# TinfoilHat0/Defending-Against-Backdoors-with-Robust-Learning-Rate

Measured on NVIDIA H100. Metric: fl_rounds_per_sec, higher is better.
Workload: dtype bf16

## Files before the change

### defending-against-backdoors-with-robust-learning-rate_b200/ops/csrc/gemm.cu

```cuda
#include <cuda.h>
#include <stdlib.h>

#include "common.cuh"
#include "gemm.h"
#include "stem_gather.cuh"
#include "wgmma.cuh"

namespace rlr {

using namespace wg;

constexpr int BM = 128;
constexpr int BK = 64;
constexpr int kConsumers = 256;
constexpr int kThreads = kConsumers + 64;
constexpr int kEpiThreads = kConsumers;

template <int BN, int kOcc = 2>
struct TileCfg {
    static_assert(kOcc != 1 || BN == 128, "the one-wave configuration exists for the 128-wide tile");
    static constexpr int kStages = kOcc == 1 ? 6 : kOcc == 3 ? (BN == 64 ? 3 : 2) : (BN == 64 ? 4 : 3);
    static constexpr int kABytes = BM * BK * 2;
    static constexpr int kBBytes = BN * BK * 2;
    static constexpr int kStageBytes = kABytes + kBBytes;
// ... 222 lines not shown
        named_bar(1, kEpiThreads);
        if (dbg && et == 0) dbg[6] = (long long)gtimer();
        constexpr int kChunks = BN * 2 / 16;
        __nv_bfloat16* out = reinterpret_cast<__nv_bfloat16*>(p.out);
        constexpr int kIters = BM * kChunks / kEpiThreads;
        constexpr int kBatch = kIters < 8 ? kIters : 8;
#pragma unroll
        for (int it0 = 0; it0 < kIters; it0 += kBatch) {
            uint4 oldv[kBatch];
            if (p.accumulate) {
#pragma unroll
                for (int j = 0; j < kBatch; ++j) {
                    const int idx = et + (it0 + j) * kEpiThreads, r = idx / kChunks, ch = idx - r * kChunks;
                    const int gi = tail->row_index[r];
                    oldv[j] = make_uint4(0, 0, 0, 0);
                    if (gi >= 0 && col0 + ch * 8 < p.N) oldv[j] = *reinterpret_cast<const uint4*>(out + (size_t)gi * p.ldc + col0 + ch * 8);
                }
            }
#pragma unroll
            for (int j = 0; j < kBatch; ++j) {
                const int idx = et + (it0 + j) * kEpiThreads, r = idx / kChunks, ch = idx - r * kChunks;
                const int gi = tail->row_index[r];
                if (gi < 0 || col0 + ch * 8 >= p.N) continue;
                uint4 val = *reinterpret_cast<const uint4*>(staging + r * Cfg::kPitch + ch * 16);
                if (p.accumulate) {
                    const __nv_bfloat162* o2 = reinterpret_cast<const __nv_bfloat162*>(&oldv[j]);
                    __nv_bfloat162* v2 = reinterpret_cast<__nv_bfloat162*>(&val);
#pragma unroll
                    for (int q = 0; q < 4; ++q) {
                        const float2 a = __bfloat1622float2(v2[q]), b = __bfloat1622float2(o2[q]);
                        v2[q] = __floats2bfloat162_rn(a.x + b.x, a.y + b.y);
                    }
                }
                *reinterpret_cast<uint4*>(out + (size_t)gi * p.ldc + col0 + ch * 8) = val;
            }
        }
        if (kStats) {
            named_bar(1, kEpiThreads);
            for (int i = et; i < 2 * BN; i += kEpiThreads)
                if (col0 + (i % BN) < p.N)
                    atomicAdd(p.stats + (size_t)(blockIdx.x % kStatSlots) * 2 * p.N + (i < BN ? 0 : p.N) + col0 + (i % BN), red[i]);
        }
        }
    }
}

typedef CUresult (*EncodeTiledFn)(CUtensorMap*, CUtensorMapDataType, cuuint32_t, void*, const cuuint64_t*, const cuuint64_t*,
                                  const cuuint32_t*, const cuuint32_t*, CUtensorMapInterleave, CUtensorMapSwizzle,
                                  CUtensorMapL2promotion, CUtensorMapFloatOOBfill);

static EncodeTiledFn get_encode_fn() {
    static EncodeTiledFn fn = nullptr;
    if (!fn) {
        void* f = nullptr;
        cudaDriverEntryPointQueryResult q;
        if (cudaGetDriverEntryPoint("cuTensorMapEncodeTiled", &f, cudaEnableDefault, &q) != cudaSuccess || !f) return nullptr;
        fn = reinterpret_cast<EncodeTiledFn>(f);
    }
    return fn;
}

cudaError_t make_tmap_bf16(CUtensorMap* map, const void* base, int rank, const uint64_t* dims, const uint64_t* strides_bytes,
                           const uint32_t* box, const uint32_t* elem_strides = nullptr) {
    EncodeTiledFn fn = get_encode_fn();
    if (!fn) return cudaErrorNotSupported;
    cuuint64_t gd[5], gs[4];
    cuuint32_t bx[5], es[5];
    for (int i = 0; i < rank; ++i) {
        gd[i] = dims[i];
        es[i] = elem_strides ? elem_strides[i] : 1;
        bx[i] = box[i] * es[i];
        if (bx[i] > 256 || es[i] < 1 || es[i] > 8) return cudaErrorInvalidValue;
    }
    for (int i = 0; i + 1 < rank; ++i) gs[i] = strides_bytes[i];
    const CUresult r = fn(map, CU_TENSOR_MAP_DATA_TYPE_BFLOAT16, (cuuint32_t)rank, const_cast<void*>(base), gd, gs, bx, es,
                          CU_TENSOR_MAP_INTERLEAVE_NONE, CU_TENSOR_MAP_SWIZZLE_128B, CU_TENSOR_MAP_L2_PROMOTION_L2_256B,
                          CU_TENSOR_MAP_FLOAT_OOB_FILL_NONE);
    return r == CUDA_SUCCESS ? cudaSuccess : cudaErrorInvalidValue;
}

template <int BN>
cudaError_t launch_persistent_bn(const CUtensorMap& tmA, const CUtensorMap& tmB, const ConvGemmParams& p, int m_tiles, int num_sms,
                                 cudaStream_t st, int occ = 1);

static int g_occ3 = -1;
void set_conv_occ3(int level) { g_occ3 = level < 0 ? 0 : (level > 1 ? 1 : level); }
static int conv_occ3() {
    if (g_occ3 < 0) { const char* e = getenv("RLR_CONV_OCC3"); set_conv_occ3(e ? atoi(e) : 1); }
    return g_occ3;
}

template <int BN, int kOcc>
static cudaError_t launch_bn_occ(const CUtensorMap& tmA, const CUtensorMap& tmB, const CUtensorMap& tmC, const ConvGemmParams& p, int m_tiles,
                                 cudaStream_t st) {
    using Cfg = TileCfg<BN, kOcc>;
    static bool configured = false;
    if (!configured) {
        RLR_CUDA_CHECK(cudaFuncSetAttribute(umma_conv_gemm_kernel<BN, false, false, kOcc>, cudaFuncAttributeMaxDynamicSharedMemorySize, Cfg::kSmemBytes));
        RLR_CUDA_CHECK(cudaFuncSetAttribute(umma_conv_gemm_kernel<BN, false, true, kOcc>, cudaFuncAttributeMaxDynamicSharedMemorySize, Cfg::kSmemBytes));
        configured = true;
    }
    dim3 grid(m_tiles, (p.N + BN - 1) / BN);
    if (p.b_mn) return launch_kernel(umma_conv_gemm_kernel<BN, false, true, kOcc>, grid, dim3(kThreads), Cfg::kSmemBytes, st, tmA, tmB, tmC, p);
    return launch_kernel(umma_conv_gemm_kernel<BN, false, false, kOcc>, grid, dim3(kThreads), Cfg::kSmemBytes, st, tmA, tmB, tmC, p);
}

static int sm_count() {
    static const int sms = [] {
        int dev = 0, n = 0;
        if (cudaGetDevice(&dev) != cudaSuccess || cudaDeviceGetAttribute(&n, cudaDevAttrMultiProcessorCount, dev) != cudaSuccess) return 132;
        return n;
    }();
    return sms;
}

static int g_persistent = -1;
void set_persistent_conv(int on) { g_persistent = on ? 1 : 0; }

static int persistent_sms() {
    if (g_persistent < 0) { const char* e = getenv("RLR_PERSISTENT_CONV"); g_persistent = (e && atoi(e) > 0) ? 1 : 0; }
    if (!g_persistent) return 0;
    static const int sms = [] {
        int dev = 0, n = 0;
        if (cudaGetDevice(&dev) != cudaSuccess || cudaDeviceGetAttribute(&n, cudaDevAttrMultiProcessorCount, dev) != cudaSuccess) return 0;
        return n;
    }();
    return sms;
}

static int g_split_prod = -1;
void set_conv_split_producer(int on) { g_split_prod = on ? 1 : 0; }
static long long* g_trace = nullptr;
void set_conv_trace(long long* buf) { g_trace = buf; }
long long* conv_trace_buf() { return g_trace; }

static int g_tma_store = -1;
void set_conv_tma_store(int on) { g_tma_store = on ? 1 : 0; }
static bool tma_store_enabled() {
    if (g_tma_store < 0) { const char* e = getenv("RLR_TMA_STORE"); g_tma_store = (e && atoi(e) == 0) ? 0 : 1; }
    return g_tma_store != 0;
}
static cudaError_t make_out_tmap(CUtensorMap* tmC, const ConvGemmParams& p) {
    if (p.ldc % 8) return cudaErrorInvalidValue;
    if (p.mode == 1) {
        const uint64_t d[4] = {(uint64_t)p.N, (uint64_t)p.Wo, (uint64_t)p.Ho, (uint64_t)p.NB};
        const uint64_t s[3] = {(uint64_t)p.out_stride * p.ldc * 2, (uint64_t)p.out_stride * p.OutW * p.ldc * 2, (uint64_t)p.OutH * p.OutW * p.ldc * 2};
        const uint32_t b[4] = {64, (uint32_t)p.TW, (uint32_t)p.TH, (uint32_t)p.TN};
        const char* base = reinterpret_cast<const char*>(p.out) + ((size_t)p.out_ph * p.OutW + p.out_pw) * p.ldc * 2;
        return make_tmap_bf16(tmC, base, 4, d, s, b);
    }
    const uint64_t d[2] = {(uint64_t)p.N, (uint64_t)p.M}, s[1] = {(uint64_t)p.ldc * 2};
    const uint32_t b[2] = {64, BM};
    return make_tmap_bf16(tmC, p.out, 2, d, s, b);
}

static void finish_params(ConvGemmParams& p, CUtensorMap& tmC) {
    p.dbg = g_trace;
    {
        static const int epi_slots = [] { const char* e = getenv("RLR_EPI_STAT_SLOTS"); int v = e ? atoi(e) : 2; return v < 1 ? 1 : (v > kStatSlots ? kStatSlots : v); }();
        p.stat_slots = epi_slots;
    }
    p.tma_store = 0;
    if (tma_store_enabled() && !p.accumulate && ((reinterpret_cast<uintptr_t>(p.out) & 15) == 0) && make_out_tmap(&tmC, p) == cudaSuccess)
        p.tma_store = 1;
    if (g_split_prod < 0) { const char* e = getenv("RLR_SPLIT_PRODUCER"); g_split_prod = (e && atoi(e) == 0) ? 0 : 1; }
    p.split_prod = (g_split_prod && !p.b_src) ? 1 : 0;
}

template <int BN>
static cudaError_t launch_bn(const CUtensorMap& tmA, const CUtensorMap& tmB, const CUtensorMap& tmC, const ConvGemmParams& p, int m_tiles,
                             cudaStream_t st) {
    using Cfg = TileCfg<BN>;
    if (p.b_src && !p.stats && p.N <= BN) {
        static const int stem_persistent = [] { const char* e = getenv("RLR_STEM_PERSISTENT"); return e ? atoi(e) : 2; }();
        if (stem_persistent && m_tiles >= 2 * sm_count())
            return launch_persistent_bn<BN>(tmA, tmB, p, m_tiles, sm_count(), st, stem_persistent == 2 ? 2 : 1);
    }
    if (!p.stats && !p.b_src && persistent_sms() > 0 && m_tiles * ((p.N + BN - 1) / BN) > persistent_sms())
        return launch_persistent_bn<BN>(tmA, tmB, p, m_tiles, persistent_sms(), st);
    if constexpr (BN == 64)
        if ((!p.stats || p.tma_store) && conv_occ3() >= 1) return launch_bn_occ<BN, 3>(tmA, tmB, tmC, p, m_tiles, st);
    static bool configured = false;
    if (!configured) {
        RLR_CUDA_CHECK(cudaFuncSetAttribute(umma_conv_gemm_kernel<BN, false, false>, cudaFuncAttributeMaxDynamicSharedMemorySize, Cfg::kSmemBytes));
        RLR_CUDA_CHECK(cudaFuncSetAttribute(umma_conv_gemm_kernel<BN, true, false>, cudaFuncAttributeMaxDynamicSharedMemorySize, Cfg::kSmemBytes));
        RLR_CUDA_CHECK(cudaFuncSetAttribute(umma_conv_gemm_kernel<BN, false, true>, cudaFuncAttributeMaxDynamicSharedMemorySize, Cfg::kSmemBytes));
        configured = true;
    }
    dim3 grid(m_tiles, (p.N + BN - 1) / BN);
    if (p.b_mn) return launch_kernel(umma_conv_gemm_kernel<BN, false, true>, grid, dim3(kThreads), Cfg::kSmemBytes, st, tmA, tmB, tmC, p);
    if (p.stats && !p.tma_store) return launch_kernel(umma_conv_gemm_kernel<BN, true, false>, grid, dim3(kThreads), Cfg::kSmemBytes, st, tmA, tmB, tmC, p);
    return launch_kernel(umma_conv_gemm_kernel<BN, false, false>, grid, dim3(kThreads), Cfg::kSmemBytes, st, tmA, tmB, tmC, p);
}

static int pick_bn(int N) { return (N % 128 == 0) ? 128 : 64; }

static int g_one_wave = 1;
void set_conv_one_wave(int on) { g_one_wave = on ? 1 : 0; }

constexpr int kOneWaveMinKb = 24;
struct ConvTile { int bn; bool one_wave; };
static ConvTile pick_conv_tile(long long px, int m_tiles, int Cout, int num_kb, bool one_wave_ok) {
    const int sms = sm_count();
    if (g_one_wave && one_wave_ok && Cout % 128 == 0 && num_kb >= kOneWaveMinKb) {
        const int ctas = m_tiles * (Cout / 128);
        if (ctas <= sms && 10 * ctas >= 9 * sms) return {128, true};
    }
    const int bn = pick_bn(Cout);
    if (bn == 128 && ((px + BM - 1) / BM) * (Cout / 128) < sms) return {64, false};
    return {bn, false};
}

cudaError_t launch_gemm_bf16(const void* A, const void* B, void* out, int M, int N, int K, int lda, int ldb, int ldc,
                             const float* bias, int relu, int accumulate, float* stats, cudaStream_t st, const DropSpec* drop) {
    if (K % BK || N % 8 || M <= 0) return cudaErrorInvalidValue;
    if (drop && drop->thr && (accumulate || stats || ldc % 8)) return cudaErrorInvalidValue;
    const int m_tiles = (M + BM - 1) / BM;
    int bn = pick_bn(N);
    {
        static const int small64 = [] { const char* e = getenv("RLR_GEMM_SMALL_BN64"); return e ? atoi(e) : 0; }();
        if (small64 && bn == 128 && m_tiles * (N / 128) < sm_count()) bn = 64;
    }
    CUtensorMap tmA, tmB;
    {
        const uint64_t d[2] = {(uint64_t)K, (uint64_t)M}, s[1] = {(uint64_t)lda * 2};
        const uint32_t b[2] = {BK, BM};
        RLR_CUDA_CHECK(make_tmap_bf16(&tmA, A, 2, d, s, b));
    }
    {
        const uint64_t d[2] = {(uint64_t)K, (uint64_t)N}, s[1] = {(uint64_t)ldb * 2};
        const uint32_t b[2] = {BK, (uint32_t)bn};
        RLR_CUDA_CHECK(make_tmap_bf16(&tmB, B, 2, d, s, b));
    }
    ConvGemmParams p{};
    p.M = M; p.N = N; p.num_kb = K / BK; p.mode = 0; p.in_stride = 1; p.out_stride = 1;
    p.out = out; p.ldc = ldc; p.bias = bias; p.stats = stats; p.relu = relu; p.accumulate = accumulate;
    if (drop && drop->thr) p.drop = *drop;
    CUtensorMap tmC = tmA;
    finish_params(p, tmC);
    return bn == 128 ? launch_bn<128>(tmA, tmB, tmC, p, m_tiles, st) : launch_bn<64>(tmA, tmB, tmC, p, m_tiles, st);
}

cudaError_t launch_stem_gemm_bf16(const void* A, const void* W, void* out, int M, int N, int kvalid, int ldw, const float* bias, int relu,
                                  float* stats, const uint32_t* wait_flags, int wait_lo, int wait_hi, const uint32_t* wait_epoch,
                                  cudaStream_t st) {
    if (N % 8 || M <= 0 || kvalid < 1 || kvalid > BK || ldw < kvalid) return cudaErrorInvalidValue;
    if (wait_flags && (!wait_epoch || wait_lo > wait_hi || wait_lo < 0)) return cudaErrorInvalidValue;
    const int m_tiles = (M + BM - 1) / BM;
    const int bn = pick_bn(N);
    CUtensorMap tmA;
    {
        const uint64_t d[2] = {(uint64_t)BK, (uint64_t)M}, s[1] = {(uint64_t)BK * 2};
        const uint32_t b[2] = {BK, BM};
        RLR_CUDA_CHECK(make_tmap_bf16(&tmA, A, 2, d, s, b));
    }
    ConvGemmParams p{};
    p.M = M; p.N = N; p.num_kb = 1; p.mode = 0; p.in_stride = 1; p.out_stride = 1;
    p.out = out; p.ldc = N; p.bias = bias; p.stats = stats; p.relu = relu; p.accumulate = 0;
    p.b_src = reinterpret_cast<const __nv_bfloat16*>(W); p.b_ld = ldw; p.b_kvalid = kvalid;
    p.wait_flags = wait_flags; p.wait_lo = wait_lo; p.wait_hi = wait_hi; p.wait_epoch = wait_epoch;
    CUtensorMap tmC = tmA;
    finish_params(p, tmC);
// ... 56 lines not shown
```

### defending-against-backdoors-with-robust-learning-rate_b200/ops/csrc/gemm.h

```cpp
#pragma once
#include <cuda_runtime.h>
#include <cuda_bf16.h>
#include <stdint.h>

#include "dropspec.h"

namespace rlr {

constexpr int kStatSlots = 16;

struct ConvGemmParams {
    int M, N, num_kb;
    int mode;
    int cblocks;
    int TW, TH, TN;
    int Ho, Wo, NB;
    int tiles_w, tiles_h;
    int ntaps;
    int in_stride;
    int out_stride, out_ph, out_pw, OutH, OutW;
    int8_t dh[9], dw[9];
    int dn[9];
    int b_mn;
    int wtap[9];
    int wcols;
    DropSpec drop;
    int tma_store;
    int split_prod;
    long long* dbg;
    const __nv_bfloat16* b_src;
    int b_ld, b_kvalid;
    const uint32_t* wait_flags;
    int wait_lo, wait_hi;
    const uint32_t* wait_epoch;
    void* out;
    int ldc;
    const float* bias;
    float* stats;
    int stat_slots;
    int relu, accumulate;
};

cudaError_t launch_gemm_bf16(const void* A, const void* B, void* out, int M, int N, int K, int lda, int ldb, int ldc,
                             const float* bias, int relu, int accumulate, float* stats, cudaStream_t st, const DropSpec* drop = nullptr);
cudaError_t launch_stem_gemm_bf16(const void* A, const void* W, void* out, int M, int N, int kvalid, int ldw, const float* bias, int relu,
                                  float* stats, const uint32_t* wait_flags, int wait_lo, int wait_hi, const uint32_t* wait_epoch,
                                  cudaStream_t st);
void set_pdl(int on);
cudaError_t launch_gemm_splitk_bf16(const void* A, const void* B, void* out, float* ws, int M, int N, int K, const float* bias, int relu,
                                    int num_sms, cudaStream_t st, const DropSpec* drop = nullptr);
void set_persistent_conv(int on);
void set_conv_occ3(int level);
void set_conv_one_wave(int on);
void set_conv_tma_store(int on);
void set_conv_split_producer(int on);
void set_conv_trace(long long* buf);
long long* conv_trace_buf();
cudaError_t launch_conv_bf16(const void* x, const void* w, void* out, int NB, int planes, int Hin, int Win, int Cin, int Ho, int Wo,
                             int Cout, int ldc, int ntaps, const int* dh, const int* dw, const int* dplane, const float* bias,
                             int relu, int accumulate, float* stats, cudaStream_t st, const int* wtap = nullptr, int w_taps_total = 0,
                             int in_stride = 1, int out_stride = 1, int out_ph = 0, int out_pw = 0);

cudaError_t launch_conv3x3_halo_bf16(const void* x, const void* w, void* out, int NB, int Hin, int Win, int H, int W, int Cout, const float* bias,
                                     int relu, int accumulate, float* stats, int bo_mode, long long* dbg, int num_sms, cudaStream_t st);

cudaError_t launch_conv3x3_halo3_bf16(const void* x, const void* w, void* out, int NB, int H, int W, int Cout, const float* bias, int relu,
                                      int accumulate, int num_sms, cudaStream_t st);

cudaError_t launch_conv_wgrad_bf16(const void* dy, const void* x, float* dW, int NB, int planes, int Hin, int Win, int Cin, int Cin_valid,
                                   int Ho, int Wo, int Cout, int ntaps, const int* dh, const int* dw, const int* dplane, int num_sms,
                                   cudaStream_t st, int in_stride = 1);
cudaError_t launch_conv_wgrad_halo_bf16(const void* dy, const void* x, float* dW, int NB, int H, int W, int Cin_valid, int Cout,
                                        int num_sms, cudaStream_t st);
void set_wgrad_rows(int on);
void wgrad_launch_counts(long long* out);
cudaError_t launch_linear_wgrad_bf16(const void* dy, const void* x, float* dW, int B, int N, int K, int num_sms, cudaStream_t st);

cudaError_t launch_ordered_sum_f32(float* out, const float* part, int nparts, long long n, cudaStream_t st);
cudaError_t launch_ordered_sum_f64(double* out, const double* part, int nparts, long long n, cudaStream_t st);
cudaError_t launch_channel_stats(const __nv_bfloat16* x, long long M, int C, float* stats , int num_sms, cudaStream_t st,
                                 int only_sum = 0, int nslots = 1);
cudaError_t launch_bn_finalize(const float* stats, int slots, float* mean_rstd, float* running_mean, float* running_var, int C,
                               float count, float eps, float momentum, int train, cudaStream_t st);
cudaError_t launch_bn_apply(const __nv_bfloat16* x, const __nv_bfloat16* res, __nv_bfloat16* y, const float* gamma, const float* beta,
                            float* mean_rstd, long long M, int C, int relu, int fin_mode, const float* stats, int slots, float count,
                            float eps, float momentum, float* running_mean, float* running_var, int num_sms, cudaStream_t st);
cudaError_t launch_bn_bwd_reduce(const __nv_bfloat16* dy, const __nv_bfloat16* y, const __nv_bfloat16* x, const float* mean_rstd,
                                 float* dsum , long long M, int C, int relu, int num_sms, cudaStream_t st,
                                 const float* gamma = nullptr, const float* beta = nullptr, int nslots = 1);
cudaError_t launch_bn_bwd_apply(const __nv_bfloat16* dy, const __nv_bfloat16* y, const __nv_bfloat16* x, const float* gamma,
                                const float* mean_rstd, const float* dsum, __nv_bfloat16* dx, __nv_bfloat16* dres, float* dgamma,
                                float* dbeta, long long M, int C, int relu, int num_sms, cudaStream_t st, const float* beta = nullptr, int nslots = 1);
cudaError_t launch_gn_fwd(const __nv_bfloat16* x, const __nv_bfloat16* res, __nv_bfloat16* y, const float* gamma, const float* beta,
                          float* mean_rstd, int B, int HW, int C, int G, float eps, int relu, int num_sms, cudaStream_t st);
cudaError_t launch_gn_bwd(const __nv_bfloat16* dy, const __nv_bfloat16* y, const __nv_bfloat16* x, const float* gamma,
                          const float* mean_rstd, __nv_bfloat16* dx, __nv_bfloat16* dres, float* dgamma, float* dbeta, int B, int HW,
                          int C, int G, int relu, int num_sms, cudaStream_t st);
cudaError_t launch_relu_bwd(__nv_bfloat16* dy, const __nv_bfloat16* y, long long n, int num_sms, cudaStream_t st, float scale = 1.0f);
cudaError_t launch_maxpool2_fwd(const __nv_bfloat16* x, __nv_bfloat16* y, uint8_t* idx, int B, int H, int W, int C, cudaStream_t st,
                                float drop_p = 0.f, uint64_t seed = 0, const long long* step = nullptr, uint64_t stream = 0);
cudaError_t launch_maxpool2_bwd(const __nv_bfloat16* dy, const uint8_t* idx, __nv_bfloat16* dx, int B, int H, int W, int C, cudaStream_t st,
                                float drop_p, uint64_t seed, const long long* step, uint64_t stream, const __nv_bfloat16* zmask);
cudaError_t launch_avgpool_fwd(const __nv_bfloat16* x, __nv_bfloat16* y, int B, int HW, int C, cudaStream_t st);
cudaError_t launch_avgpool_bwd(const __nv_bfloat16* dy, __nv_bfloat16* dx, int B, int HW, int C, cudaStream_t st);
cudaError_t launch_dropout_fwd(const __nv_bfloat16* x, __nv_bfloat16* y, uint8_t* mask, long long n, float p, uint64_t seed,
                               const long long* step, uint64_t stream, cudaStream_t st);
cudaError_t launch_dropout_bwd(const __nv_bfloat16* dy, const uint8_t* mask, __nv_bfloat16* dx, long long n, float p, cudaStream_t st);
cudaError_t launch_space_to_depth(const __nv_bfloat16* x, __nv_bfloat16* y, int NB, int H, int W, int C, int num_sms, cudaStream_t st);
cudaError_t launch_im2col_small(const __nv_bfloat16* x, __nv_bfloat16* A, int NB, int H, int W, int C, int Ho, int Wo, int k, int pad,
                                int num_sms, cudaStream_t st);
cudaError_t launch_depth_to_space(const __nv_bfloat16* x4, __nv_bfloat16* y, int NB, int H, int W, int C, int accumulate, int plane_mask,
                                  int num_sms, cudaStream_t st);
cudaError_t launch_filter_gather_transpose(const __nv_bfloat16* w, __nv_bfloat16* wt, int Cout, int T, int Cin, int nsub, const int* taps,
                                           cudaStream_t st);
cudaError_t launch_filter_transpose(const __nv_bfloat16* w, __nv_bfloat16* wt, int Cout, int ntaps, int Cin, cudaStream_t st);
cudaError_t launch_linear_small_fwd(const __nv_bfloat16* x, const __nv_bfloat16* w, const float* bias, __nv_bfloat16* y, int B, int K,
                                    int N, int relu, cudaStream_t st);
cudaError_t launch_linear_small_fwd2(const __nv_bfloat16* x, const __nv_bfloat16* w, const float* bias, __nv_bfloat16* y, int B, int K,
                                     int N, int relu, cudaStream_t st);
cudaError_t launch_linear_small_bwd2(const __nv_bfloat16* x, const __nv_bfloat16* dy, const __nv_bfloat16* w, __nv_bfloat16* dx,
                                     float* dw, float* db, int B, int K, int N, int accumulate_dx, cudaStream_t st);
cudaError_t launch_linear_small_bwd(const __nv_bfloat16* x, const __nv_bfloat16* dy, const __nv_bfloat16* w, __nv_bfloat16* dx,
                                    float* dw, float* db, int B, int K, int N, int accumulate_dx, cudaStream_t st);

}
```

### defending-against-backdoors-with-robust-learning-rate_b200/ops/csrc/gemm_binding.cpp

```cpp
#include <torch/extension.h>
#include <ATen/cuda/CUDAContext.h>
#include <c10/cuda/CUDAGuard.h>
#include <c10/cuda/CUDAStream.h>
#include <c10/cuda/CUDACachingAllocator.h>

#include <vector>

#include "gemm.h"

namespace rlr {
void* scratch_alloc(size_t bytes, cudaStream_t st) {
    return c10::cuda::CUDACachingAllocator::raw_alloc_with_stream(bytes < 256 ? 256 : bytes, st);
}
void scratch_free(void* p) { c10::cuda::CUDACachingAllocator::raw_delete(p); }
}

namespace {
inline cudaStream_t cur_stream() { return c10::cuda::getCurrentCUDAStream().stream(); }
inline int num_sms() { return at::cuda::getCurrentDeviceProperties()->multiProcessorCount; }
inline void check(cudaError_t e, const char* what) { TORCH_CHECK(e == cudaSuccess, what, ": ", cudaGetErrorString(e)); }
template <typename T>
inline T* opt(const c10::optional<at::Tensor>& t) { return t.has_value() && t->defined() ? reinterpret_cast<T*>(t->data_ptr()) : nullptr; }
inline const __nv_bfloat16* bf(const at::Tensor& t) {
    TORCH_CHECK(t.is_cuda() && t.scalar_type() == at::kBFloat16 && t.is_contiguous(), "expected contiguous CUDA bf16 tensor");
// ... 254 lines not shown
}
void maxpool2_bwd(at::Tensor dy, at::Tensor idx, at::Tensor dx, double drop_p, int64_t drop_seed, c10::optional<at::Tensor> drop_step, int64_t drop_stream,
                  c10::optional<at::Tensor> relu_out) {
    c10::cuda::CUDAGuard g(dx.device());
    const rlr::DropSpec d = drop_spec(drop_p, drop_seed, drop_step, drop_stream);
    const bool zm = relu_out.has_value() && relu_out->defined();
    TORCH_CHECK(!zm || (relu_out->scalar_type() == at::kBFloat16 && relu_out->is_contiguous() && relu_out->numel() == dy.numel()), "relu_out must match dy");
    TORCH_CHECK(dy.is_contiguous() && dx.is_contiguous() && idx.is_contiguous() && dy.size(1) == dx.size(1) / 2 && dy.size(2) == dx.size(2) / 2);
    check(rlr::launch_maxpool2_bwd(bf(dy), (const uint8_t*)idx.data_ptr(), bfm(dx), dx.size(0), dx.size(1), dx.size(2), dx.size(3), cur_stream(),
                                   (float)drop_p, d.seed, d.step, d.stream, zm ? bf(*relu_out) : nullptr), "maxpool2_bwd");
}
void avgpool_fwd(at::Tensor x, at::Tensor y) {
    c10::cuda::CUDAGuard g(x.device());
    check(rlr::launch_avgpool_fwd(bf(x), bfm(y), x.size(0), x.size(1) * x.size(2), x.size(3), cur_stream()), "avgpool_fwd");
}
void avgpool_bwd(at::Tensor dy, at::Tensor dx) {
    c10::cuda::CUDAGuard g(dx.device());
    check(rlr::launch_avgpool_bwd(bf(dy), bfm(dx), dx.size(0), dx.size(1) * dx.size(2), dx.size(3), cur_stream()), "avgpool_bwd");
}
void dropout_fwd(at::Tensor x, at::Tensor y, at::Tensor mask, double p, int64_t seed, at::Tensor step, int64_t stream) {
    c10::cuda::CUDAGuard g(x.device());
    check(rlr::launch_dropout_fwd(bf(x), bfm(y), (uint8_t*)mask.data_ptr(), x.numel(), (float)p, (uint64_t)seed,
                                  (const long long*)step.data_ptr(), (uint64_t)stream, cur_stream()), "dropout_fwd");
}
void dropout_bwd(at::Tensor dy, at::Tensor mask, at::Tensor dx, double p) {
    c10::cuda::CUDAGuard g(dx.device());
    check(rlr::launch_dropout_bwd(bf(dy), (const uint8_t*)mask.data_ptr(), bfm(dx), dx.numel(), (float)p, cur_stream()), "dropout_bwd");
}
void space_to_depth(at::Tensor x, at::Tensor y) {
    c10::cuda::CUDAGuard g(x.device());
    check(rlr::launch_space_to_depth(bf(x), bfm(y), x.size(0), x.size(1), x.size(2), x.size(3), num_sms(), cur_stream()), "space_to_depth");
}
void im2col_small(at::Tensor x, at::Tensor A, int64_t k, int64_t pad) {
    c10::cuda::CUDAGuard g(x.device());
    const int NB = x.size(0), H = x.size(1), W = x.size(2), C = x.size(3);
    const int Ho = H + 2 * pad - k + 1, Wo = W + 2 * pad - k + 1;
    TORCH_CHECK(x.dim() == 4 && x.is_contiguous() && A.is_contiguous() && A.numel() == (int64_t)NB * Ho * Wo * 64, "im2col_small: A must be [NB*Ho*Wo, 64]");
    check(rlr::launch_im2col_small(bf(x), bfm(A), NB, H, W, C, Ho, Wo, (int)k, (int)pad, num_sms(), cur_stream()), "im2col_small");
}
void depth_to_space(at::Tensor x4, at::Tensor y, bool accumulate, int64_t plane_mask) {
    c10::cuda::CUDAGuard g(y.device());
    check(rlr::launch_depth_to_space(bf(x4), bfm(y), y.size(0), y.size(1), y.size(2), y.size(3), accumulate, (int)plane_mask, num_sms(),
                                     cur_stream()), "depth_to_space");
}
void filter_gather_transpose(at::Tensor w, at::Tensor wt, int64_t Cout, int64_t T, int64_t Cin, std::vector<int64_t> taps) {
    c10::cuda::CUDAGuard g(w.device());
    int t[9];
    TORCH_CHECK(taps.size() >= 1 && taps.size() <= 9);
    for (size_t i = 0; i < taps.size(); ++i) t[i] = (int)taps[i];
    check(rlr::launch_filter_gather_transpose(bf(w), bfm(wt), Cout, T, Cin, (int)taps.size(), t, cur_stream()), "filter_gather_transpose");
}
void filter_transpose(at::Tensor w, at::Tensor wt, int64_t Cout, int64_t ntaps, int64_t Cin) {
    c10::cuda::CUDAGuard g(w.device());
    check(rlr::launch_filter_transpose(bf(w), bfm(wt), Cout, ntaps, Cin, cur_stream()), "filter_transpose");
}
void linear_small_fwd(at::Tensor x, at::Tensor w, c10::optional<at::Tensor> bias, at::Tensor y, bool relu) {
    c10::cuda::CUDAGuard g(x.device());
    check(rlr::launch_linear_small_fwd(bf(x), bf(w), opt<const float>(bias), bfm(y), x.size(0), x.size(1), w.size(0), relu, cur_stream()), "linear_small_fwd");
}
void linear_small_bwd(at::Tensor x, at::Tensor dy, at::Tensor w, c10::optional<at::Tensor> dx, at::Tensor dw, c10::optional<at::Tensor> db,
                      bool accumulate_dx) {
    c10::cuda::CUDAGuard g(x.device());
    check(rlr::launch_linear_small_bwd(bf(x), bf(dy), bf(w), const_cast<__nv_bfloat16*>(bfo(dx)), (float*)dw.data_ptr(), opt<float>(db),
                                       x.size(0), x.size(1), w.size(0), accumulate_dx, cur_stream()), "linear_small_bwd");
}
void linear_small_fwd2(at::Tensor x, at::Tensor w, c10::optional<at::Tensor> bias, at::Tensor y, bool relu) {
    c10::cuda::CUDAGuard g(x.device());
    check(rlr::launch_linear_small_fwd2(bf(x), bf(w), opt<const float>(bias), bfm(y), x.size(0), x.size(1), w.size(0), relu, cur_stream()), "linear_small_fwd2");
}
void linear_small_bwd2(at::Tensor x, at::Tensor dy, at::Tensor w, c10::optional<at::Tensor> dx, at::Tensor dw, c10::optional<at::Tensor> db,
                       bool accumulate_dx) {
    c10::cuda::CUDAGuard g(x.device());
    check(rlr::launch_linear_small_bwd2(bf(x), bf(dy), bf(w), const_cast<__nv_bfloat16*>(bfo(dx)), (float*)dw.data_ptr(), opt<float>(db),
                                        x.size(0), x.size(1), w.size(0), accumulate_dx, cur_stream()), "linear_small_bwd2");
}
}

void register_gemm_bindings(py::module_& m) {
    m.attr("STAT_SLOTS") = rlr::kStatSlots;
    m.def("set_persistent_conv", [](bool on) { rlr::set_persistent_conv(on ? 1 : 0); });
    m.def("set_pdl", [](bool on) { rlr::set_pdl(on ? 1 : 0); });
    m.def("set_conv_occ3", [](int64_t level) { rlr::set_conv_occ3((int)level); });
    m.def("set_conv_one_wave", [](bool on) { rlr::set_conv_one_wave(on ? 1 : 0); });
    m.def("set_wgrad_rows", [](bool on) { rlr::set_wgrad_rows(on ? 1 : 0); });
    m.def("wgrad_launch_counts", [] {
        long long c[3];
        rlr::wgrad_launch_counts(c);
        return std::vector<int64_t>{c[0], c[1], c[2]};
    });
    m.def("set_conv_tma_store", [](bool on) { rlr::set_conv_tma_store(on ? 1 : 0); });
    m.def("set_conv_split_producer", [](bool on) { rlr::set_conv_split_producer(on ? 1 : 0); });
    m.def("set_conv_trace", [](c10::optional<at::Tensor> buf) {
        rlr::set_conv_trace(buf.has_value() && buf->defined() ? reinterpret_cast<long long*>(buf->data_ptr<int64_t>()) : nullptr);
    });
    m.def("gemm_bf16", &gemm_bf16, py::arg("A"), py::arg("B"), py::arg("out"), py::arg("bias"), py::arg("relu"), py::arg("accumulate"), py::arg("stats"),
          py::arg("drop_p") = 0.0, py::arg("drop_seed") = 0, py::arg("drop_step") = py::none(), py::arg("drop_stream") = 0);
    m.def("stem_gemm_bf16", &stem_gemm_bf16, py::arg("A"), py::arg("W"), py::arg("out"), py::arg("bias"), py::arg("relu"), py::arg("stats"),
          py::arg("ready_ptr") = 0, py::arg("lo") = 0, py::arg("hi") = 0, py::arg("epoch") = py::none());
    m.def("gemm_splitk_bf16", &gemm_splitk_bf16, py::arg("A"), py::arg("B"), py::arg("out"), py::arg("ws"), py::arg("bias"), py::arg("relu"),
          py::arg("drop_p") = 0.0, py::arg("drop_seed") = 0, py::arg("drop_step") = py::none(), py::arg("drop_stream") = 0);
    m.def("conv_bf16", &conv_bf16);
    m.def("conv_bf16_strided", &conv_bf16_strided);
    m.def("conv_wgrad_bf16_strided", &conv_wgrad_bf16_strided);
    m.def("conv3x3_halo_bf16", &conv3x3_halo_bf16);
    m.def("conv3x3_halo3_bf16", &conv3x3_halo3_bf16);
    m.def("conv_wgrad_bf16", &conv_wgrad_bf16);
    m.def("linear_wgrad_bf16", &linear_wgrad_bf16);
    m.def("conv_wgrad_halo_bf16", &conv_wgrad_halo_bf16);
    m.def("channel_stats", &channel_stats);
    m.def("ordered_sum", &ordered_sum);
    m.def("bias_grad", &bias_grad);
    m.def("bn_finalize", &bn_finalize);
    m.def("bn_apply", &bn_apply);
    m.def("bn_bwd", &bn_bwd);
    m.def("bn_bwd_recompute", &bn_bwd_recompute);
    m.def("gn_fwd", &gn_fwd);
    m.def("gn_bwd", &gn_bwd);
    m.def("relu_bwd", &relu_bwd, py::arg("dy"), py::arg("y"), py::arg("scale") = 1.0);
    m.def("maxpool2_fwd", &maxpool2_fwd, py::arg("x"), py::arg("y"), py::arg("idx"), py::arg("drop_p") = 0.0, py::arg("drop_seed") = 0,
          py::arg("drop_step") = py::none(), py::arg("drop_stream") = 0);
    m.def("maxpool2_bwd", &maxpool2_bwd, py::arg("dy"), py::arg("idx"), py::arg("dx"), py::arg("drop_p") = 0.0, py::arg("drop_seed") = 0,
          py::arg("drop_step") = py::none(), py::arg("drop_stream") = 0, py::arg("relu_out") = py::none());
    m.def("avgpool_fwd", &avgpool_fwd);
    m.def("avgpool_bwd", &avgpool_bwd);
    m.def("dropout_fwd", &dropout_fwd);
    m.def("dropout_bwd", &dropout_bwd);
    m.def("space_to_depth", &space_to_depth);
    m.def("im2col_small", &im2col_small);
    m.def("filter_transpose", &filter_transpose);
    m.def("depth_to_space", &depth_to_space);
    m.def("filter_gather_transpose", &filter_gather_transpose);
    m.def("linear_small_fwd", &linear_small_fwd);
    m.def("linear_small_bwd", &linear_small_bwd);
    m.def("linear_small_fwd2", &linear_small_fwd2);
    m.def("linear_small_bwd2", &linear_small_bwd2);
}
```

### defending-against-backdoors-with-robust-learning-rate_b200/ops/csrc/gemm_persistent.cu

```cuda
#include <cuda.h>

#include "common.cuh"
#include "gemm.h"
#include "stem_gather.cuh"
#include "wgmma.cuh"

namespace rlr {

using namespace wg;

constexpr int PBM = 128, PBK = 64, PConsumers = 256, PThreads = PConsumers + 32;

template <int BN, int kOcc = 1>
struct PCfg {
    static constexpr int kStages = kOcc == 2 ? 3 : (BN == 64 ? 7 : 5);
    static constexpr int kABytes = PBM * PBK * 2;
    static constexpr int kBBytes = BN * PBK * 2;
    static constexpr int kStageBytes = kABytes + kBBytes;
    static constexpr int kPitch = BN * 2 + 16;
    static constexpr int kStagingBytes = PBM * kPitch;
    static constexpr int kRingBytes = kStages * kStageBytes;
    static constexpr int kTailBytes = BN == 128 ? 2048 : 1024;
    static constexpr int kSmemBytes = kRingBytes + kStagingBytes + 1024 + kTailBytes;
};

struct __align__(8) PShared {
    uint64_t full[8];
    uint64_t empty[8];
    int row_index[PBM];
};
static_assert(sizeof(PShared) <= 704, "the bias slice starts 704 bytes into the tail");

template <int BN, bool kBMN, int kOcc = 1>
__global__ void __launch_bounds__(PThreads, kOcc)
umma_conv_gemm_persistent_kernel(const __grid_constant__ CUtensorMap tmA, const __grid_constant__ CUtensorMap tmB, const ConvGemmParams p,
                                  const int m_tiles, const int total_tiles) {
    using Cfg = PCfg<BN, kOcc>;
    extern __shared__ uint8_t smem_raw[];
    uint8_t* smem = reinterpret_cast<uint8_t*>((reinterpret_cast<uintptr_t>(smem_raw) + 1023) & ~uintptr_t(1023));
    uint8_t* staging = smem + Cfg::kRingBytes;
    PShared* sh = reinterpret_cast<PShared*>(staging + Cfg::kStagingBytes);
    const int warp = threadIdx.x >> 5, lane = threadIdx.x & 31;

    if (warp == 8 && lane == 0) {
        prefetch_tmap(&tmA); prefetch_tmap(&tmB);
        for (int s = 0; s < Cfg::kStages; ++s) { mbar_init(&sh->full[s], 1); mbar_init(&sh->empty[s], 8); }
        fence_barrier_init();
    }
    __syncthreads();

    auto origin = [&](int tile, int& tile_m, int& tile_n, int& n0, int& h0, int& w0) {
        tile_m = tile % m_tiles; tile_n = tile / m_tiles;
        n0 = h0 = w0 = 0;
        if (p.mode == 1) {
            const int tw_i = tile_m % p.tiles_w, th_i = (tile_m / p.tiles_w) % p.tiles_h, tn_i = tile_m / (p.tiles_w * p.tiles_h);
            w0 = tw_i * p.TW; h0 = th_i * p.TH; n0 = tn_i * p.TN;
        }
    };

    if (warp == 8) {
        if (p.b_src) stem_gather_b(p, smem + Cfg::kABytes, BN, 0, lane);
        if (lane == 0) {
            int stage = 0;
            uint32_t phase = 0;
            for (int tile = blockIdx.x; tile < total_tiles; tile += gridDim.x) {
                int tile_m, tile_n, n0, h0, w0;
                origin(tile, tile_m, tile_n, n0, h0, w0);
                for (int kb = 0; kb < p.num_kb; ++kb) {
                    mbar_wait(&sh->empty[stage], phase ^ 1);
                    uint8_t* sa = smem + stage * Cfg::kStageBytes;
                    uint8_t* sb = sa + Cfg::kABytes;
                    mbar_expect_tx(&sh->full[stage], p.b_src ? Cfg::kABytes : Cfg::kStageBytes);
                    const int tap = p.mode == 1 ? kb / p.cblocks : 0, cb = p.mode == 1 ? kb - tap * p.cblocks : 0;
                    if (p.mode == 1) tma_load_4d(&tmA, &sh->full[stage], sa, cb * PBK, w0 * p.in_stride + p.dw[tap], h0 * p.in_stride + p.dh[tap],
                                                n0 + p.dn[tap]);
                    else tma_load_2d(&tmA, &sh->full[stage], sa, kb * PBK, tile_m * PBM);
                    if (p.b_src) {
                    } else if (kBMN) {
                        for (int g = 0; g < BN / 64; ++g)
                            tma_load_2d(&tmB, &sh->full[stage], sb + g * 8192, p.wtap[tap] * p.wcols + tile_n * BN + g * 64, cb * PBK);
                    } else {
                        tma_load_2d(&tmB, &sh->full[stage], sb, kb * PBK, tile_n * BN);
                    }
// ... 40 lines not shown
#pragma unroll
            for (int i = 0; i < BN / 2; ++i) acc[i] = 0.f;
            consumer_mainloop<BN, Cfg::kStages, Cfg::kStageBytes, Cfg::kABytes, kBMN>(acc, smem, sh->full, sh->empty, p.num_kb,
                                                                                       (uint32_t)wgi * 64 * 128, b_fixed, stage, phase, lane);
            named_bar(1, PConsumers);
#pragma unroll
            for (int j = 0; j < BN / 8; ++j) {
                const int c = frag_col(t, 4 * j);
#pragma unroll
                for (int h = 0; h < 2; ++h) {
                    float a = acc[4 * j + 2 * h], b = acc[4 * j + 2 * h + 1];
                    if (p.bias) { a += bias_s[c]; b += bias_s[c + 1]; }
                    if (p.relu) { a = fmaxf(a, 0.f); b = fmaxf(b, 0.f); }
                    *reinterpret_cast<uint32_t*>(staging + (r0 + 8 * h) * Cfg::kPitch + c * 2) = pack_bf16x2(a, b);
                }
            }
            named_bar(1, PConsumers);
#pragma unroll
            for (int it0 = 0; it0 < kIters; it0 += kBatch) {
                uint4 oldv[kBatch];
                if (p.accumulate) {
#pragma unroll
                    for (int j = 0; j < kBatch; ++j) {
                        const int idx = et + (it0 + j) * PConsumers, r = idx / kChunks, ch = idx - r * kChunks;
                        const int gi = sh->row_index[r];
                        oldv[j] = make_uint4(0, 0, 0, 0);
                        if (gi >= 0 && col0 + ch * 8 < p.N) oldv[j] = *reinterpret_cast<const uint4*>(out + (size_t)gi * p.ldc + col0 + ch * 8);
                    }
                }
#pragma unroll
                for (int j = 0; j < kBatch; ++j) {
                    const int idx = et + (it0 + j) * PConsumers, r = idx / kChunks, ch = idx - r * kChunks;
                    const int gi = sh->row_index[r];
                    if (gi < 0 || col0 + ch * 8 >= p.N) continue;
                    uint4 val = *reinterpret_cast<const uint4*>(staging + r * Cfg::kPitch + ch * 16);
                    if (p.accumulate) {
                        const __nv_bfloat162* o2 = reinterpret_cast<const __nv_bfloat162*>(&oldv[j]);
                        __nv_bfloat162* v2 = reinterpret_cast<__nv_bfloat162*>(&val);
#pragma unroll
                        for (int q = 0; q < 4; ++q) {
                            const float2 a = __bfloat1622float2(v2[q]), b = __bfloat1622float2(o2[q]);
                            v2[q] = __floats2bfloat162_rn(a.x + b.x, a.y + b.y);
                        }
                    }
                    *reinterpret_cast<uint4*>(out + (size_t)gi * p.ldc + col0 + ch * 8) = val;
                }
            }
            named_bar(1, PConsumers);
        }
    }
}

template <int BN>
cudaError_t launch_persistent_bn(const CUtensorMap& tmA, const CUtensorMap& tmB, const ConvGemmParams& p, int m_tiles, int num_sms,
                                 cudaStream_t st, int occ) {
    const int n_tiles = (p.N + BN - 1) / BN;
    const int total = m_tiles * n_tiles;
    if (occ == 2 && !p.b_mn) {
        using Cfg = PCfg<BN, 2>;
        static bool configured2 = false;
        if (!configured2) {
            RLR_CUDA_CHECK(cudaFuncSetAttribute(umma_conv_gemm_persistent_kernel<BN, false, 2>, cudaFuncAttributeMaxDynamicSharedMemorySize, Cfg::kSmemBytes));
            configured2 = true;
        }
        const int grid = total < 2 * num_sms ? total : 2 * num_sms;
        umma_conv_gemm_persistent_kernel<BN, false, 2><<<grid, PThreads, Cfg::kSmemBytes, st>>>(tmA, tmB, p, m_tiles, total);
        return cudaGetLastError();
    }
    using Cfg = PCfg<BN>;
    static bool configured = false;
    if (!configured) {
        RLR_CUDA_CHECK(cudaFuncSetAttribute(umma_conv_gemm_persistent_kernel<BN, false>, cudaFuncAttributeMaxDynamicSharedMemorySize, Cfg::kSmemBytes));
        RLR_CUDA_CHECK(cudaFuncSetAttribute(umma_conv_gemm_persistent_kernel<BN, true>, cudaFuncAttributeMaxDynamicSharedMemorySize, Cfg::kSmemBytes));
        configured = true;
    }
    const int grid = total < num_sms ? total : num_sms;
    if (p.b_mn) umma_conv_gemm_persistent_kernel<BN, true><<<grid, PThreads, Cfg::kSmemBytes, st>>>(tmA, tmB, p, m_tiles, total);
    else umma_conv_gemm_persistent_kernel<BN, false><<<grid, PThreads, Cfg::kSmemBytes, st>>>(tmA, tmB, p, m_tiles, total);
    return cudaGetLastError();
}
template cudaError_t launch_persistent_bn<64>(const CUtensorMap&, const CUtensorMap&, const ConvGemmParams&, int, int, cudaStream_t, int);
template cudaError_t launch_persistent_bn<128>(const CUtensorMap&, const CUtensorMap&, const ConvGemmParams&, int, int, cudaStream_t, int);

}
```

Measured before the change: 0.7313.

## Add persistent ping-pong warp-specialized conv GEMM with dynamic tile scheduler

Adds a persistent conv GEMM kernel with one producer warpgroup and two consumer warpgroups that alternate tiles (ping-pong). Each consumer's epilogue overlaps with the other's mainloop, and register budgets are rebalanced with setmaxnreg. Tiles are handed out through an atomic counter that resets itself at the end of each launch. It is on by default for mode-1 convs without stats or b_src when there are at least two waves of tiles. The counter, keyed per output pointer, could race if two launches with the same output buffer run concurrently on different streams.

```diff
diff --git a/defending-against-backdoors-with-robust-learning-rate_b200/ops/csrc/gemm.cu b/defending-against-backdoors-with-robust-learning-rate_b200/ops/csrc/gemm.cu
--- a/defending-against-backdoors-with-robust-learning-rate_b200/ops/csrc/gemm.cu
+++ b/defending-against-backdoors-with-robust-learning-rate_b200/ops/csrc/gemm.cu
@@ -328,6 +328,9 @@
 template <int BN>
 cudaError_t launch_persistent_bn(const CUtensorMap& tmA, const CUtensorMap& tmB, const ConvGemmParams& p, int m_tiles, int num_sms,
                                  cudaStream_t st, int occ = 1);
+template <int BN>
+cudaError_t launch_pingpong_bn(const CUtensorMap& tmA, const CUtensorMap& tmB, const CUtensorMap& tmC, const ConvGemmParams& p, int m_tiles,
+                               int num_sms, cudaStream_t st);
 
 static int g_occ3 = -1;
 void set_conv_occ3(int level) { g_occ3 = level < 0 ? 0 : (level > 1 ? 1 : level); }
@@ -374,6 +377,12 @@
     return sms;
 }
 
+static int g_pingpong = 1;
+void set_conv_pingpong(int level) { g_pingpong = level < 0 ? 0 : (level > 2 ? 2 : level); }
+static bool pingpong_takes(const ConvGemmParams& p, int tiles) {
+    return g_pingpong && p.mode == 1 && !p.stats && !p.b_src && (g_pingpong == 2 || tiles >= 2 * sm_count());
+}
+
 static int g_split_prod = -1;
 void set_conv_split_producer(int on) { g_split_prod = on ? 1 : 0; }
 static long long* g_trace = nullptr;
@@ -424,6 +433,7 @@
     }
     if (!p.stats && !p.b_src && persistent_sms() > 0 && m_tiles * ((p.N + BN - 1) / BN) > persistent_sms())
         return launch_persistent_bn<BN>(tmA, tmB, p, m_tiles, persistent_sms(), st);
+    if (pingpong_takes(p, m_tiles * ((p.N + BN - 1) / BN))) return launch_pingpong_bn<BN>(tmA, tmB, tmC, p, m_tiles, sm_count(), st);
     if constexpr (BN == 64)
         if ((!p.stats || p.tma_store) && conv_occ3() >= 1) return launch_bn_occ<BN, 3>(tmA, tmB, tmC, p, m_tiles, st);
     static bool configured = false;
diff --git a/defending-against-backdoors-with-robust-learning-rate_b200/ops/csrc/gemm.h b/defending-against-backdoors-with-robust-learning-rate_b200/ops/csrc/gemm.h
--- a/defending-against-backdoors-with-robust-learning-rate_b200/ops/csrc/gemm.h
+++ b/defending-against-backdoors-with-robust-learning-rate_b200/ops/csrc/gemm.h
@@ -52,6 +52,8 @@
 void set_persistent_conv(int on);
 void set_conv_occ3(int level);
 void set_conv_one_wave(int on);
+void set_conv_pingpong(int level);
+long long conv_pingpong_launches();
 void set_conv_tma_store(int on);
 void set_conv_split_producer(int on);
 void set_conv_trace(long long* buf);
diff --git a/defending-against-backdoors-with-robust-learning-rate_b200/ops/csrc/gemm_binding.cpp b/defending-against-backdoors-with-robust-learning-rate_b200/ops/csrc/gemm_binding.cpp
--- a/defending-against-backdoors-with-robust-learning-rate_b200/ops/csrc/gemm_binding.cpp
+++ b/defending-against-backdoors-with-robust-learning-rate_b200/ops/csrc/gemm_binding.cpp
@@ -360,6 +360,8 @@
     m.def("set_pdl", [](bool on) { rlr::set_pdl(on ? 1 : 0); });
     m.def("set_conv_occ3", [](int64_t level) { rlr::set_conv_occ3((int)level); });
     m.def("set_conv_one_wave", [](bool on) { rlr::set_conv_one_wave(on ? 1 : 0); });
+    m.def("set_conv_pingpong", [](int64_t level) { rlr::set_conv_pingpong((int)level); });
+    m.def("conv_pingpong_launches", [] { return (int64_t)rlr::conv_pingpong_launches(); });
     m.def("set_wgrad_rows", [](bool on) { rlr::set_wgrad_rows(on ? 1 : 0); });
     m.def("wgrad_launch_counts", [] {
         long long c[3];
diff --git a/defending-against-backdoors-with-robust-learning-rate_b200/ops/csrc/gemm_persistent.cu b/defending-against-backdoors-with-robust-learning-rate_b200/ops/csrc/gemm_persistent.cu
--- a/defending-against-backdoors-with-robust-learning-rate_b200/ops/csrc/gemm_persistent.cu
+++ b/defending-against-backdoors-with-robust-learning-rate_b200/ops/csrc/gemm_persistent.cu
@@ -1,4 +1,8 @@
 #include <cuda.h>
+
+#include <map>
+#include <mutex>
+#include <utility>
 
 #include "common.cuh"
 #include "gemm.h"
@@ -205,4 +209,303 @@
 template cudaError_t launch_persistent_bn<64>(const CUtensorMap&, const CUtensorMap&, const ConvGemmParams&, int, int, cudaStream_t, int);
 template cudaError_t launch_persistent_bn<128>(const CUtensorMap&, const CUtensorMap&, const ConvGemmParams&, int, int, cudaStream_t, int);
 
-}
+constexpr int PPThreads = 384;
+
+template <int BN>
+struct PPCfg {
+    static constexpr int kStages = BN == 64 ? 6 : 4;
+    static constexpr int kABytes = PBM * PBK * 2;
+    static constexpr int kBBytes = BN * PBK * 2;
+    static constexpr int kStageBytes = kABytes + kBBytes;
+    static constexpr int kRingBytes = kStages * kStageBytes;
+    static constexpr int kStagingBytes = PBM * BN * 2;
+};
+
+constexpr int kTileQ = 4;
+
+struct __align__(8) PPShared {
+    uint64_t full[8];
+    uint64_t empty[8];
+    uint64_t tile_full[kTileQ];
+    uint64_t tile_empty[kTileQ];
+    int tile_id[kTileQ];
+    int row_index[2][PBM];
+    float bias[2][128];
+};
+
+template <int BN>
+constexpr int pp_smem_bytes() { return PPCfg<BN>::kRingBytes + 2 * PPCfg<BN>::kStagingBytes + 1024  + (int)sizeof(PPShared); }
+
+template <uint32_t N>
+__device__ __forceinline__ void setmaxnreg_dec() { asm volatile("setmaxnreg.dec.sync.aligned.u32 %0;" ::"n"(N)); }
+template <uint32_t N>
+__device__ __forceinline__ void setmaxnreg_inc() { asm volatile("setmaxnreg.inc.sync.aligned.u32 %0;" ::"n"(N)); }
+__device__ __forceinline__ void named_bar_arrive(int id, int threads) { asm volatile("bar.arrive %0, %1;" ::"r"(id), "r"(threads) : "memory"); }
+
+template <int BN, int kStages, int kStageBytes, int kABytes, bool kBMN>
+__device__ __forceinline__ int pingpong_mainloop(float (&acc0)[BN / 2], float (&acc1)[BN / 2], uint8_t* smem, uint64_t* full,
+                                                 uint64_t* empty, int num_kb, int stage, uint32_t phase, int lane) {
+    int prev = -1;
+    for (int kb = 0; kb < num_kb; ++kb) {
+        mbar_wait(&full[stage], phase);
+        const uint32_t sa = smem_u32(smem + stage * kStageBytes);
+        const uint32_t sb = sa + kABytes;
+        wgmma_fence();
+#pragma unroll
+        for (int k = 0; k < 4; ++k) {
+            const uint64_t db = kBMN ? smem_desc_sw128(sb + k * 2048, 8192, 1024) : smem_desc_sw128(sb + k * 32, 16, 1024);
+            const uint32_t scale_d = (kb > 0 || k > 0) ? 1u : 0u;
+            wgmma_bf16<BN, 0, kBMN ? 1 : 0>(acc0, smem_desc_sw128(sa + k * 32, 16, 1024), db, scale_d);
+            wgmma_bf16<BN, 0, kBMN ? 1 : 0>(acc1, smem_desc_sw128(sa + 64 * 128 + k * 32, 16, 1024), db, scale_d);
+        }
+        wgmma_commit();
+        wgmma_wait<1>();
+        if (prev >= 0 && lane == 0) mbar_arrive(&empty[prev]);
+        prev = stage;
+        if (++stage == kStages) { stage = 0; phase ^= 1; }
+    }
+    return prev;
+}
+
+template <int BN>
+__device__ __forceinline__ void pingpong_drain(float (&acc0)[BN / 2], float (&acc1)[BN / 2], uint64_t* empty, int last, int lane) {
+    wgmma_wait<0>();
+    fence_acc(acc0);
+    fence_acc(acc1);
+    if (last >= 0 && lane == 0) mbar_arrive(&empty[last]);
+}
+
+template <int BN>
+__device__ __forceinline__ void pp_stage_rows(const float (&acc)[BN / 2], uint8_t* staging, int row0, int t, const float* bias_s, bool has_bias,
+                                              int relu) {
+#pragma unroll
+    for (int j = 0; j < BN / 8; ++j) {
+        const int col = frag_col(t, 4 * j);
+#pragma unroll
+        for (int h = 0; h < 2; ++h) {
+            const int row = row0 + frag_row(t, 0) + 8 * h;
+            float a = acc[4 * j + 2 * h], b = acc[4 * j + 2 * h + 1];
+            if (has_bias) { a += bias_s[col]; b += bias_s[col + 1]; }
+            if (relu) { a = fmaxf(a, 0.f); b = fmaxf(b, 0.f); }
+            *reinterpret_cast<uint32_t*>(staging + (col >> 6) * (PBM * 128) + row * 128 + ((((col & 63) >> 3) ^ (row & 7)) << 4) + (col & 7) * 2) =
+                pack_bf16x2(a, b);
+        }
+    }
+}
+
+template <int BN, bool kBMN>
+__global__ void __launch_bounds__(PPThreads, 1)
+umma_conv_gemm_pingpong_kernel(const __grid_constant__ CUtensorMap tmA, const __grid_constant__ CUtensorMap tmB,
+                               const __grid_constant__ CUtensorMap tmC, const ConvGemmParams p, const int m_tiles, const int total_tiles,
+                               int* tile_counter) {
+    using Cfg = PPCfg<BN>;
+    extern __shared__ uint8_t smem_raw[];
+    uint8_t* smem = reinterpret_cast<uint8_t*>((reinterpret_cast<uintptr_t>(smem_raw) + 1023) & ~uintptr_t(1023));
+    uint8_t* staging_base = smem + Cfg::kRingBytes;
+    PPShared* sh = reinterpret_cast<PPShared*>(staging_base + 2 * Cfg::kStagingBytes);
+    const int wgi = threadIdx.x >> 7, t = threadIdx.x & 127, lane = threadIdx.x & 31;
+
+    if (threadIdx.x == 0) {
+        prefetch_tmap(&tmA); prefetch_tmap(&tmB);
+        if (p.tma_store) prefetch_tmap(&tmC);
+        for (int s = 0; s < Cfg::kStages; ++s) { mbar_init(&sh->full[s], 1); mbar_init(&sh->empty[s], 4); }
+        for (int s = 0; s < kTileQ; ++s) { mbar_init(&sh->tile_full[s], 1); mbar_init(&sh->tile_empty[s], 128); }
+        fence_barrier_init();
+    }
+    __syncthreads();
+    pdl_wait();
+    pdl_trigger();
+
+    auto origin = [&](int tile, int& tile_n, int& n0, int& h0, int& w0) {
+        const int tile_m = tile % m_tiles;
+        tile_n = tile / m_tiles;
+        const int tw_i = tile_m % p.tiles_w, th_i = (tile_m / p.tiles_w) % p.tiles_h, tn_i = tile_m / (p.tiles_w * p.tiles_h);
+        w0 = tw_i * p.TW; h0 = th_i * p.TH; n0 = tn_i * p.TN;
+    };
+
+    if (wgi == 0) {
+        setmaxnreg_dec<40>();
+        if (t == 0) {
+            auto publish = [&](int q, int tile) {
+                mbar_wait(&sh->tile_empty[q % kTileQ], ((q / kTileQ) & 1) ^ 1);
+                sh->tile_id[q % kTileQ] = tile;
+                mbar_arrive(&sh->tile_full[q % kTileQ]);
+            };
+            int stage = 0;
+            uint32_t phase = 0;
+            int tile = blockIdx.x;
+            publish(0, tile);
+            for (int q = 0; tile >= 0; ++q) {
+                const int drawn = atomicAdd(tile_counter, 1);
+                if (drawn == total_tiles - 1) atomicExch(tile_counter, 0);
+                int next = (int)gridDim.x + drawn;
+                if (next >= total_tiles) next = -1;
+                publish(q + 1, next);
+                int tile_n, n0, h0, w0;
+                origin(tile, tile_n, n0, h0, w0);
+                for (int kb = 0; kb < p.num_kb; ++kb) {
+                    mbar_wait(&sh->empty[stage], phase ^ 1);
+                    uint8_t* sa = smem + stage * Cfg::kStageBytes;
+                    uint8_t* sb = sa + Cfg::kABytes;
+                    mbar_expect_tx(&sh->full[stage], Cfg::kStageBytes);
+                    const int tap = kb / p.cblocks, cb = kb - tap * p.cblocks;
+                    tma_load_4d(&tmA, &sh->full[stage], sa, cb * PBK, w0 * p.in_stride + p.dw[tap], h0 * p.in_stride + p.dh[tap], n0 + p.dn[tap]);
+                    if (kBMN) {
+                        for (int g = 0; g < BN / 64; ++g)
+                            tma_load_2d(&tmB, &sh->full[stage], sb + g * 8192, p.wtap[tap] * p.wcols + tile_n * BN + g * 64, cb * PBK);
+                    } else {
+                        tma_load_2d(&tmB, &sh->full[stage], sb, kb * PBK, tile_n * BN);
+                    }
+                    if (++stage == Cfg::kStages) { stage = 0; phase ^= 1; }
+                }
+                if (next < 0) publish(q + 2, -1);
+                tile = next;
+            }
+        }
+        return;
+    }
+
+    setmaxnreg_inc<232>();
+    const int c = wgi - 1;
+    uint8_t* staging = staging_base + c * Cfg::kStagingBytes;
+    int* row_index = sh->row_index[c];
+    float* bias_s = sh->bias[c];
+    const int epi_bar = 1 + c;
+    const int my_turn = 3 + c, other_turn = 4 - c;
+    const bool has_bias = !kBMN && p.bias != nullptr;
+    __nv_bfloat16* out = reinterpret_cast<__nv_bfloat16*>(p.out);
+    int bias_tile_n = -1;
+    for (int q = c;; q += 2) {
+        mbar_wait(&sh->tile_full[q % kTileQ], (uint32_t)(q / kTileQ) & 1u);
+        const int tile = sh->tile_id[q % kTileQ];
+        if (tile < 0) break;
+        int tile_n, n0, h0, w0;
+        origin(tile, tile_n, n0, h0, w0);
+        const int col0 = tile_n * BN;
+        {
+            const int tw = t % p.TW, th = (t / p.TW) % p.TH, tn = t / (p.TW * p.TH);
+            const int w = w0 + tw, h = h0 + th, n = n0 + tn;
+            row_index[t] = (w < p.Wo && h < p.Ho && n < p.NB) ? ((n * p.OutH + h * p.out_stride + p.out_ph) * p.OutW + w * p.out_stride + p.out_pw) : -1;
+        }
+        if (has_bias && tile_n != bias_tile_n) {
+            for (int i = t; i < BN; i += 128) bias_s[i] = (col0 + i < p.N) ? p.bias[col0 + i] : 0.f;
+            bias_tile_n = tile_n;
+        }
+        float acc0[BN / 2], acc1[BN / 2];
+#pragma unroll
+        for (int i = 0; i < BN / 2; ++i) { acc0[i] = 0.f; acc1[i] = 0.f; }
+        if (q > 0) named_bar(my_turn, 256);
+        const int pos = q * p.num_kb;
+        const int last = pingpong_mainloop<BN, Cfg::kStages, Cfg::kStageBytes, Cfg::kABytes, kBMN>(
+            acc0, acc1, smem, sh->full, sh->empty, p.num_kb, pos % Cfg::kStages, (uint32_t)(pos / Cfg::kStages) & 1u, lane);
+        mbar_wait(&sh->tile_full[(q + 1) % kTileQ], (uint32_t)((q + 1) / kTileQ) & 1u);
+        if (sh->tile_id[(q + 1) % kTileQ] >= 0) named_bar_arrive(other_turn, 256);
+        mbar_arrive(&sh->tile_empty[q % kTileQ]);
+        pingpong_drain<BN>(acc0, acc1, sh->empty, last, lane);
+        if (p.tma_store && t == 0) tma_store_wait_read();
+        named_bar(epi_bar, 128);
+        pp_stage_rows<BN>(acc0, staging, 0, t, bias_s, has_bias, p.relu);
+        pp_stage_rows<BN>(acc1, staging, 64, t, bias_s, has_bias, p.relu);
+        if (p.tma_store) {
+            fence_proxy_async_smem();
+            named_bar(epi_bar, 128);
+            if (t == 0) {
+#pragma unroll
+                for (int g = 0; g < BN / 64; ++g) {
+                    if (col0 + g * 64 >= p.N) break;
+                    tma_store_4d(&tmC, staging + g * (PBM * 128), col0 + g * 64, w0, h0, n0);
+                }
+                tma_store_commit();
+            }
+        } else {
+            named_bar(epi_bar, 128);
+            constexpr int kChunks = BN * 2 / 16;
+            constexpr int kIters = PBM * kChunks / 128;
+            constexpr int kBatch = 8;
+#pragma unroll
+            for (int it0 = 0; it0 < kIters; it0 += kBatch) {
+                uint4 oldv[kBatch];
+                if (p.accumulate) {
+#pragma unroll
+                    for (int j = 0; j < kBatch; ++j) {
+                        const int idx = t + (it0 + j) * 128, r = idx / kChunks, ch = idx - r * kChunks;
+                        const int gi = row_index[r];
+                        oldv[j] = make_uint4(0, 0, 0, 0);
+                        if (gi >= 0 && col0 + ch * 8 < p.N) oldv[j] = *reinterpret_cast<const uint4*>(out + (size_t)gi * p.ldc + col0 + ch * 8);
+                    }
+                }
+#pragma unroll
+                for (int j = 0; j < kBatch; ++j) {
+                    const int idx = t + (it0 + j) * 128, r = idx / kChunks, ch = idx - r * kChunks;
+                    const int gi = row_index[r];
+                    if (gi < 0 || col0 + ch * 8 >= p.N) continue;
+                    uint4 val = *reinterpret_cast<const uint4*>(staging + (ch >> 3) * (PBM * 128) + r * 128 + (((ch & 7) ^ (r & 7)) << 4));
+                    if (p.accumulate) {
+                        const __nv_bfloat162* o2 = reinterpret_cast<const __nv_bfloat162*>(&oldv[j]);
+                        __nv_bfloat162* v2 = reinterpret_cast<__nv_bfloat162*>(&val);
+#pragma unroll
+                        for (int qq = 0; qq < 4; ++qq) {
+                            const float2 a = __bfloat1622float2(v2[qq]), b = __bfloat1622float2(o2[qq]);
+                            v2[qq] = __floats2bfloat162_rn(a.x + b.x, a.y + b.y);
+                        }
+                    }
+                    *reinterpret_cast<uint4*>(out + (size_t)gi * p.ldc + col0 + ch * 8) = val;
+                }
+            }
+            named_bar(epi_bar, 128);
+        }
+    }
+    if (p.tma_store && t == 0) tma_store_wait_read();
+}
+
+static long long g_pingpong_launches = 0;
+
+constexpr int kPPCounters = 4096;
+__device__ int g_pp_counters[kPPCounters];
+
+static int* pp_counter(const void* out) {
+    static std::mutex mu;
+    static std::map<std::pair<int, const void*>, int> slot;
+    static int* base[64] = {};
+    int dev = 0;
+    if (cudaGetDevice(&dev) != cudaSuccess || dev >= 64) return nullptr;
+    std::lock_guard<std::mutex> lock(mu);
+    if (!base[dev] && cudaGetSymbolAddress(reinterpret_cast<void**>(&base[dev]), g_pp_counters) != cudaSuccess) return nullptr;
+    auto it = slot.find({dev, out});
+    if (it == slot.end()) {
+        int used = 0;
+        for (const auto& kv : slot) used += kv.first.first == dev;
+        if (used >= kPPCounters) return nullptr;
+        it = slot.emplace(std::make_pair(dev, out), used).first;
+    }
+    return base[dev] + it->second;
+}
+long long conv_pingpong_launches() { return g_pingpong_launches; }
+
+template <int BN>
+cudaError_t launch_pingpong_bn(const CUtensorMap& tmA, const CUtensorMap& tmB, const CUtensorMap& tmC, const ConvGemmParams& p, int m_tiles,
+                               int num_sms, cudaStream_t st) {
+    if (p.mode != 1 || p.stats || p.b_src) return cudaErrorInvalidValue;
+    constexpr int kSmem = pp_smem_bytes<BN>();
+    static bool configured = false;
+    if (!configured) {
+        RLR_CUDA_CHECK(cudaFuncSetAttribute(umma_conv_gemm_pingpong_kernel<BN, false>, cudaFuncAttributeMaxDynamicSharedMemorySize, kSmem));
+        RLR_CUDA_CHECK(cudaFuncSetAttribute(umma_conv_gemm_pingpong_kernel<BN, true>, cudaFuncAttributeMaxDynamicSharedMemorySize, kSmem));
+        configured = true;
+    }
+    const int total = m_tiles * ((p.N + BN - 1) / BN);
+    const dim3 grid(total < num_sms ? total : num_sms);
+    auto launch = [&](int* ctr) {
+        ++g_pingpong_launches;
+        if (p.b_mn) return launch_kernel(umma_conv_gemm_pingpong_kernel<BN, true>, grid, dim3(PPThreads), kSmem, st, tmA, tmB, tmC, p, m_tiles, total, ctr);
+        return launch_kernel(umma_conv_gemm_pingpong_kernel<BN, false>, grid, dim3(PPThreads), kSmem, st, tmA, tmB, tmC, p, m_tiles, total, ctr);
+    };
+    if (int* ctr = pp_counter(p.out)) return launch(ctr);
+    Scratch spare(sizeof(int), st);
+    RLR_CUDA_CHECK(cudaMemsetAsync(spare.p, 0, sizeof(int), st));
+    return launch(static_cast<int*>(spare.p));
+}
+template cudaError_t launch_pingpong_bn<64>(const CUtensorMap&, const CUtensorMap&, const CUtensorMap&, const ConvGemmParams&, int, int, cudaStream_t);
+template cudaError_t launch_pingpong_bn<128>(const CUtensorMap&, const CUtensorMap&, const CUtensorMap&, const ConvGemmParams&, int, int, cudaStream_t);
+
+}
```

After: 0.7456, median of 6. +2.0%, better.
